# ZHENGXi-git/TC-VIML

Hardware: NVIDIA B200
Metric: linearized_factors_per_s (higher is better)
Workload: dtype f64

## Files before the change

tc-viml_b200/csrc/assemble2.cuh:

```cuda
#pragma once

namespace stream {

constexpr int PMAX = 12;
constexpr int FMAXP = 4096;
constexpr int PT = 64;
constexpr int PT_MAX = 512;
constexpr int TASK_T = 180;
constexpr int TASK_F = 24;
constexpr int LTASK = 32;
constexpr int AW = 4;
constexpr int LACC_W = 14;
constexpr int STAGE_D = 1024;
constexpr int LACC_D = TASK_F * LACC_W;
constexpr int WORK_D = STAGE_D + LACC_D + 192;

struct PlanPtrs {
  int4* hdr;
  int4* tasks;
  uint32_t* slots;
  uint32_t* finfo;
  uint32_t* lslots;
  int* any_irregular;
};

__host__ __device__ inline int task_base(int a0_rel, int w, int F) { return a0_rel / 64 + w * (F / TASK_F + PMAX + 4); }

__device__ __forceinline__ int warp_incl_scan(int v, int lane) {
#pragma unroll
  for (int d = 1; d < 32; d <<= 1) {
    const int t = __shfl_up_sync(0xffffffffu, v, d);
    if (lane >= d) v += t;
  }
  return v;
}

__global__ void __launch_bounds__(PT_MAX) plan_kernel(LinearizeArgs A, PlanPtrs PL) {
  extern __shared__ __align__(16) unsigned char plan_raw[];
  __shared__ int gcount[PMAX + 2], grun[PMAX + 2], lcount[PMAX + 1], lrun[PMAX + 1];
  __shared__ int s_bad, s_big, s_ntasks, s_nlslots;
  const int tid = threadIdx.x, lane = tid & 31, warp = tid >> 5, w = blockIdx.x;
  const int P = A.P, F = A.F, NTH = (int)blockDim.x;
  uint32_t* fmask = reinterpret_cast<uint32_t*>(plan_raw);
  uint32_t* fanchor = fmask + F;
  uint32_t* cexcl = fanchor + F;
  uint16_t* ford = reinterpret_cast<uint16_t*>(cexcl + F + 1);
  uint16_t* fid = ford + ((F + 1) & ~1);
  const int a0 = A.pf_window_offset[w], nf = A.pf_window_offset[w + 1] - a0;
  const int b0 = A.NL > 0 ? A.lf_window_offset[w] : 0, nl = A.NL > 0 ? A.lf_window_offset[w + 1] - b0 : 0;
  const int a0r = a0 - (int)A.pf_begin, b0r = b0 - (int)A.lf_begin;
  for (int f = tid; f < F; f += NTH) fmask[f] = 0u, fanchor[f] = 0xffu;
  for (int e = tid; e < F * P; e += NTH) fid[e] = 0xffff;
  if (tid < PMAX + 2) gcount[tid] = 0;
  if (tid < PMAX + 1) lcount[tid] = 0;
  if (tid == 0) s_bad = s_big = (nf > 65534 || nl > 65534 || nf < 0 || nl < 0) ? 1 : 0, s_ntasks = 0, s_nlslots = 0;
  __syncthreads();
  const int nfs = s_big ? 0 : nf;
  for (int k = tid; k < nfs; k += NTH) {
    const uint32_t ix = A.pf_idx[a0 + k];
    const int i = ix & 0xff, j = (ix >> 8) & 0xff, l = ix >> 16;
    if (i >= P || j >= P || l >= F || i == j) {
      s_bad = 1;
      continue;
    }
    const uint32_t old = atomicOr(&fmask[l], 1u << j);
    const uint32_t an = atomicCAS(&fanchor[l], 0xffu, (uint32_t)i);
    if (((old >> j) & 1u) || (an != 0xffu && an != (uint32_t)i)) s_bad = 1;
    fid[l * P + j] = (uint16_t)k;
  }
  __syncthreads();
  if (s_bad) {
    if (tid == 0) {
      PL.hdr[w] = make_int4(0, 0, 1, 0);
      atomicOr(PL.any_irregular, 1);
    }
    return;
  }
  uint32_t* lsl = PL.lslots + 2 * (size_t)b0r;
  if (warp == 0) {
    for (int f0 = 0; f0 < F; f0 += 32) {
      const int f = f0 + lane;
      const int key = f < F ? (fanchor[f] == 0xffu ? P : (int)fanchor[f]) : 64 + lane;
      const unsigned m = __match_any_sync(0xffffffffu, key);
      if (f < F && (m & ((1u << lane) - 1u)) == 0u) gcount[key] += __popc(m);
      __syncwarp();
    }
    {
      const int c = lane <= P ? gcount[lane] : 0;
      const int inc = warp_incl_scan(c, lane);
      if (lane <= P) grun[lane] = inc - c;
    }
    __syncwarp();
    for (int f0 = 0; f0 < F; f0 += 32) {
      const int f = f0 + lane;
      const int key = f < F ? (fanchor[f] == 0xffu ? P : (int)fanchor[f]) : 64 + lane;
      const unsigned m = __match_any_sync(0xffffffffu, key);
      const int rank = __popc(m & ((1u << lane) - 1u));
      if (f < F) ford[grun[key] + rank] = (uint16_t)f;
      __syncwarp();
      if (f < F && rank == 0) grun[key] += __popc(m);
      __syncwarp();
    }
    int carry = 0;
    for (int p0 = 0; p0 < F; p0 += 32) {
      const int p = p0 + lane;
      const int c = p < F ? __popc(fmask[ford[p]]) : 0;
      const int inc = warp_incl_scan(c, lane);
      if (p < F) cexcl[p] = (uint32_t)(carry + inc - c);
      carry += __shfl_sync(0xffffffffu, inc, 31);
    }
    if (lane == 0) cexcl[F] = (uint32_t)carry;
    __syncwarp();
    const int tb = task_base(a0r, w, F);
    int pos = 0, t = 0;
    bool at_group_start = true;
    while (pos < F) {
      const int p = pos + lane;
      const int c = p < F ? (int)(cexcl[p + 1] - cexcl[p]) : 0x10000;
      const int inc = warp_incl_scan(c, lane);
      const unsigned okm = __ballot_sync(0xffffffffu, inc <= TASK_T && p < F && lane < TASK_F);
      int n = okm == 0xffffffffu ? 32 : __ffs(~okm) - 1;
      n = max(n, 1);
      n = min(n, F - pos);
      const int an = p < F ? (fanchor[ford[p]] == 0xffu ? P : (int)fanchor[ford[p]]) : -1;
      const unsigned same = __ballot_sync(0xffffffffu, an == __shfl_sync(0xffffffffu, an, 0));
      const int na = same == 0xffffffffu ? 33 : __ffs(~same) - 1;
      int excl = 0;
      if (na <= n) {
        n = na;
        excl = at_group_start ? 1 : 0;
        at_group_start = true;
      } else {
        at_group_start = false;
      }
      if (lane == 0) PL.tasks[tb + t] = make_int4(2 * (int)cexcl[pos], 0, pos, n | (excl << 16));
      pos += n, ++t;
    }
    if (lane == 0) s_ntasks = t;
  } else if (warp == 1 && nl > 0) {
    bool bad = false;
    for (int k0 = 0; k0 < nl; k0 += 32) {
      const int k = k0 + lane;
      int key = k < nl ? A.lf_frame[b0 + k] : 64 + lane;
      if (k < nl && (key < 0 || key >= P)) bad = true, key = 96 + lane;
      const unsigned m = __match_any_sync(0xffffffffu, key);
      if (k < nl && key < P && (m & ((1u << lane) - 1u)) == 0u) lcount[key] += __popc(m);
      __syncwarp();
    }
    if (__any_sync(0xffffffffu, bad)) {
      if (lane == 0) s_bad = 1;
    } else {
      const int c = lane < P ? ((lcount[lane] + 1) & ~1) : 0;
      const int inc = warp_incl_scan(c, lane);
      if (lane < P) {
        lrun[lane] = inc - c;
        if (lcount[lane] & 1) lsl[inc - 1] = 0xffffu | ((uint32_t)lane << 16);
      }
      if (lane == 31) s_nlslots = inc;
      __syncwarp();
      for (int k0 = 0; k0 < nl; k0 += 32) {
        const int k = k0 + lane;
        const int key = k < nl ? A.lf_frame[b0 + k] : 64 + lane;
        const unsigned m = __match_any_sync(0xffffffffu, key);
        const int rank = __popc(m & ((1u << lane) - 1u));
        if (k < nl) lsl[lrun[key] + rank] = (uint32_t)k | ((uint32_t)key << 16);
        __syncwarp();
        if (k < nl && rank == 0) lrun[key] += __popc(m);
        __syncwarp();
      }
    }
  }
  __syncthreads();
  if (s_bad) {
    if (tid == 0) {
      PL.hdr[w] = make_int4(0, 0, 1, 0);
      atomicOr(PL.any_irregular, 1);
    }
    return;
  }
  const int tb = task_base(a0r, w, F), nt = s_ntasks;
  uint32_t* sl_w = PL.slots + 2 * (size_t)a0r;
  for (int t = warp; t < nt; t += NTH / 32) {
    int4 tk = PL.tasks[tb + t];
    const int p = tk.z + lane;
    const bool on = lane < (tk.w & 0xffff);
    const int l = on ? ford[p] : 0;
    const uint32_t m = on ? fmask[l] : 0u;
    const int an = (on && m) ? (int)fanchor[l] : 0xff;
    if (on) PL.finfo[(size_t)w * F + p] = (uint32_t)l | (m << 16) | ((uint32_t)(an & 15) << 28);
    uint32_t* sl = sl_w + tk.x;
    int off = 0;
    const unsigned lt = (1u << lane) - 1u;
    unsigned im = __reduce_or_sync(0xffffffffu, an < P ? 1u << an : 0u);
    while (im) {
      const int i = __ffs(im) - 1;
      im &= im - 1;
      unsigned jm = __reduce_or_sync(0xffffffffu, an == i ? m : 0u);
      while (jm) {
        const int j = __ffs(jm) - 1;
        jm &= jm - 1;
        const bool mine = an == i && ((m >> j) & 1u);
        const unsigned b = __ballot_sync(0xffffffffu, mine);
        const int n = __popc(b);
        const uint32_t key = ((uint32_t)i << 21) | ((uint32_t)j << 25);
        if (mine) sl[off + __popc(b & lt)] = (uint32_t)fid[l * P + j] | ((uint32_t)lane << 16) | key;
        if ((n & 1) && lane == 0) sl[off + n] = 0xffffu | key;
        off += (n + 1) & ~1;
      }
    }
    if (lane == 0) PL.tasks[tb + t].y = off;
  }
  if (tid == 0) PL.hdr[w] = make_int4(nt, s_nlslots, 0, 0);
}

enum Kind { K_LL = 0, K_HH, K_LH, K_LE, K_HE, K_EE, K_BL, K_BH, K_BE, K_NKIND };

struct Tables {
  uint32_t seg[128];
  uint32_t lo[64];
  uint32_t ee[32];
  uint32_t line[32];
};

constexpr uint32_t tab_entry(int R, int C, int kind, int off, bool neg) {
  const int tile = (R < 8 && C < 8) ? 0 : (R < 8 ? 1 : 2);
  return 0x80000000u | (uint32_t)(tile * 64 + (R & 7) * 8 + (C & 7)) | ((uint32_t)kind << 8) | ((uint32_t)off << 12) |
         (neg ? (1u << 18) : 0u);
}

constexpr int col_type(int c) { return c < 3 ? 0 : (c < 6 ? 1 : (c < 9 ? 2 : (c < 15 ? 3 : 4))); }
constexpr int col_sub(int c) { return c < 3 ? c : (c < 6 ? c - 3 : (c < 9 ? c - 6 : (c < 15 ? c - 9 : 0))); }

constexpr Tables make_tables() {
  Tables T{};
  int ns = 0, nlo = 0, nli = 0, nee = 0;
  constexpr int kind_order[K_NKIND] = {K_LL, K_LE, K_BL, K_EE, K_BE, K_HH, K_HE, K_BH, K_LH};
  for (int ko = 0; ko < K_NKIND; ++ko)
    for (int off = 0; off < 36; ++off) {
      const int kind = kind_order[ko];
      const bool vec = kind >= K_BL;
      if (vec && off >= 6) continue;
      const int dr = vec ? off : off / 6, dc = vec ? 0 : off % 6;
      for (int R = 0; R < 16; ++R)
        for (int C = R; C < 16; ++C) {
          const int tr = col_type(R), tc = col_type(C), r = col_sub(R), c = col_sub(C);
          bool hit = false, neg = false;
          if (tr == 0 && tc == 0) {
            if (kind == K_LL || kind == K_HH) hit = dr == r && dc == c;
            if (kind == K_LH) hit = dr == r && dc == c, neg = true;
          } else if (tr == 0 && tc == 1) {
            if (kind == K_LL) hit = dr == r && dc == 3 + c;
            if (kind == K_LH) hit = dr == 3 + c && dc == r, neg = true;
          } else if (tr == 0 && tc == 2) {
            if (kind == K_LH) hit = dr == r && dc == 3 + c;
            if (kind == K_HH) hit = dr == r && dc == 3 + c, neg = true;
          } else if (tr == 0 && tc == 3) {
            if (kind == K_LE) hit = dr == r && dc == c;
            if (kind == K_HE) hit = dr == r && dc == c, neg = true;
          } else if (tr == 0 && tc == 4) {
            if (kind == K_BL) hit = dr == r;
            if (kind == K_BH) hit = dr == r, neg = true;
          } else if (tr == 1 && tc == 1) {
            if (kind == K_LL) hit = dr == 3 + r && dc == 3 + c;
          } else if (tr == 1 && tc == 2) {
            if (kind == K_LH) hit = dr == 3 + r && dc == 3 + c;
          } else if (tr == 1 && tc == 3) {
            if (kind == K_LE) hit = dr == 3 + r && dc == c;
          } else if (tr == 1 && tc == 4) {
            if (kind == K_BL) hit = dr == 3 + r;
          } else if (tr == 2 && tc == 2) {
            if (kind == K_HH) hit = dr == 3 + r && dc == 3 + c;
          } else if (tr == 2 && tc == 3) {
            if (kind == K_HE) hit = dr == 3 + r && dc == c;
          } else if (tr == 2 && tc == 4) {
            if (kind == K_BH) hit = dr == 3 + r;
          } else if (tr == 3 && tc == 3) {
            if (kind == K_EE) hit = dr == r && dc == c;
          } else if (tr == 3 && tc == 4) {
            if (kind == K_BE) hit = dr == r;
          }
          if (!hit) continue;
          const bool per_segment = kind == K_HH || kind == K_LH || kind == K_HE || kind == K_BH;
          if (per_segment) {
            T.seg[ns++] = tab_entry(R, C, kind, off, neg);
          } else if (kind == K_EE || kind == K_BE) {
            T.ee[nee++] = tab_entry(R, C, kind, off, neg);
          } else {
            T.lo[nlo++] = tab_entry(R, C, kind, off, neg);
          }
        }
    }
  for (int r = 0; r < 6; ++r)
    for (int c = r; c < 6; ++c) T.line[nli++] = tab_entry(r, c, K_LL, r * 6 + c, false);
  for (int r = 0; r < 6; ++r) T.line[nli++] = tab_entry(r, 6, K_BL, r, false);
  return T;
}
__device__ const Tables g_tables = make_tables();
static_assert(make_tables().seg[95] != 0u && make_tables().seg[96] == 0u, "63 hi-role + 33 (lo, hi) per-segment destinations = three full rounds");
static_assert(make_tables().lo[62] != 0u && make_tables().lo[63] == 0u, "63 per-anchor destinations");
static_assert(make_tables().ee[26] != 0u && make_tables().ee[27] == 0u, "27 extrinsic destinations");
static_assert(make_tables().line[26] != 0u && make_tables().line[27] == 0u, "27 line destinations");


__device__ __forceinline__ void dmma(double& d0, double& d1, double a, double b) {
  asm volatile("mma.sync.aligned.m8n8k4.row.col.f64.f64.f64.f64 {%0,%1}, {%2}, {%3}, {%0,%1};"
               : "+d"(d0), "+d"(d1)
               : "d"(a), "d"(b));
}

__device__ __forceinline__ int blk(int br, int bc, int NB) { return br * NB - (br * (br - 1)) / 2 + (bc - br); }

__device__ __forceinline__ int swz(int f) { return ((f & 1) << 2) ^ ((f >> 1) & 3); }

struct Dest {
  int src;
  int off;
  int kind;
  unsigned sign;
};
__device__ __forceinline__ Dest decode(uint32_t e) {
  Dest d;
  d.src = (e >> 31) ? (int)(e & 0xff) : -1;
  d.off = (e >> 12) & 63;
  d.kind = (e >> 8) & 15;
  d.sign = ((e >> 18) & 1u) << 31;
  return d;
}
template <int ROUNDS>
__device__ __forceinline__ void scatter(const double* __restrict__ patch, const Dest* tab, double* __restrict__ Hc,
                                        int mybase, bool store_lh = false) {
  double v[ROUNDS];
  double* dst[ROUNDS];
#pragma unroll
  for (int r = 0; r < ROUNDS; ++r) {
    const int base = __shfl_sync(0xffffffffu, mybase, tab[r].kind);
    dst[r] = Hc + base + tab[r].off;
    const double x = patch[tab[r].src >= 0 ? tab[r].src : 0];
    v[r] = __hiloint2double(__double2hiint(x) ^ (int)tab[r].sign, __double2loint(x));
  }
#pragma unroll
  for (int r = 0; r < ROUNDS; ++r) {
    if (tab[r].src >= 0) {
      if (store_lh && tab[r].kind == K_LH) *dst[r] = v[r];
      else atomicAdd(dst[r], v[r]);
    }
  }
}

__device__ __forceinline__ int kind_base(int rs, int cs, bool isb, int lo, int hi, int NB, int boff) {
  const int e = NB - 1;
  const int x = rs == 0 ? lo : (rs == 1 ? hi : e), y = cs == 0 ? lo : (cs == 1 ? hi : e);
  return isb ? boff + 6 * x : blk(x, y, NB) * 36;
}

__device__ __forceinline__ void put_patch(double* __restrict__ patch, int lane, const double (&G)[6]) {
  double2* p2 = reinterpret_cast<double2*>(patch);
  const int o = (lane >> 2) * 4 + (lane & 3);
  p2[o] = make_double2(G[0], G[1]);
  p2[32 + o] = make_double2(G[2], G[3]);
  p2[64 + o] = make_double2(G[4], G[5]);
}

template <bool MODE_A>
__global__ void __maxnreg__(168) assemble_kernel(LinearizeArgs A, PlanPtrs PL, int use_tma) {
  extern __shared__ __align__(16) unsigned char asm_raw[];
  __shared__ int s_next;
// ... 418 lines not shown
```

tc-viml_b200/csrc/linearize_kernels.cu:

```cuda
#include <cstdlib>
#include <vector>

#include "common.cuh"

namespace {

__device__ __forceinline__ void quat_to_rot(double w, double x, double y, double z, double* R) {
  const double tx = 2.0 * x, ty = 2.0 * y, tz = 2.0 * z;
  const double twx = tx * w, twy = ty * w, twz = tz * w;
  const double txx = tx * x, txy = ty * x, txz = tz * x;
  const double tyy = ty * y, tyz = tz * y, tzz = tz * z;
  R[0] = 1.0 - (tyy + tzz);
  R[1] = txy - twz;
  R[2] = txz + twy;
  R[3] = txy + twz;
  R[4] = 1.0 - (txx + tzz);
  R[5] = tyz - twx;
  R[6] = txz - twy;
  R[7] = tyz + twx;
  R[8] = 1.0 - (txx + tyy);
}

__device__ __forceinline__ void mul_AtBt(const double* A, const double* B, double* C) {
#pragma unroll
// ... 303 lines not shown
    for (int c = 0; c < 6; ++c) {
      const double v = X[0][r] * Y[0][c] + X[1][r] * Y[1][c];
      atomicAdd(H + (size_t)(r0 + r) * D + c0 + c, v);
      if (!diag) atomicAdd(H + (size_t)(c0 + c) * D + r0 + r, v);
    }
}

__device__ __forceinline__ void point_atomics(const LinearizeArgs& A, int w, int i, int j, int f, const PointJac& J, bool live,
                                              bool warp_window) {
  const int D = A.D;
  double* H = A.out.H_pp + (size_t)w * D * D;
  double* bp = A.out.b_p + (size_t)w * D;
  const int oi = 6 * i, oj = 6 * j, oe = 6 * A.P;
  if (warp_window) {
    double v[27];
    int n = 0;
#pragma unroll
    for (int r = 0; r < 6; ++r)
#pragma unroll
      for (int c = r; c < 6; ++c) v[n++] = live ? J.c[0][r] * J.c[0][c] + J.c[1][r] * J.c[1][c] : 0.0;
#pragma unroll
    for (int r = 0; r < 6; ++r) v[21 + r] = live ? J.c[0][r] * J.r[0] + J.c[1][r] * J.r[1] : 0.0;
#pragma unroll
    for (int e = 0; e < 27; ++e)
#pragma unroll
      for (int d = 16; d > 0; d >>= 1) v[e] += __shfl_xor_sync(0xffffffffu, v[e], d);
    if ((threadIdx.x & 31) == 0) {
      n = 0;
#pragma unroll
      for (int r = 0; r < 6; ++r)
#pragma unroll
        for (int c = r; c < 6; ++c) {
          atomicAdd(H + (size_t)(oe + r) * D + oe + c, v[n]);
          if (c != r) atomicAdd(H + (size_t)(oe + c) * D + oe + r, v[n]);
          ++n;
        }
#pragma unroll
      for (int r = 0; r < 6; ++r) atomicAdd(bp + oe + r, v[21 + r]);
    }
  }
  if (!live) return;
  double* Hl = A.out.H_lp + ((size_t)w * A.F + f) * D;
  atomic_block(H, D, oi, oi, J.a, J.a, true);
  atomic_block(H, D, oi, oj, J.a, J.b, false);
  atomic_block(H, D, oi, oe, J.a, J.c, false);
  atomic_block(H, D, oj, oj, J.b, J.b, true);
  atomic_block(H, D, oj, oe, J.b, J.c, false);
  if (!warp_window) atomic_block(H, D, oe, oe, J.c, J.c, true);
#pragma unroll
  for (int r = 0; r < 6; ++r) {
    atomicAdd(bp + oi + r, J.a[0][r] * J.r[0] + J.a[1][r] * J.r[1]);
    atomicAdd(bp + oj + r, J.b[0][r] * J.r[0] + J.b[1][r] * J.r[1]);
    if (!warp_window) atomicAdd(bp + oe + r, J.c[0][r] * J.r[0] + J.c[1][r] * J.r[1]);
    atomicAdd(Hl + oi + r, J.a[0][r] * J.d[0] + J.a[1][r] * J.d[1]);
    atomicAdd(Hl + oj + r, J.b[0][r] * J.d[0] + J.b[1][r] * J.d[1]);
    atomicAdd(Hl + oe + r, J.c[0][r] * J.d[0] + J.c[1][r] * J.d[1]);
  }
  atomicAdd(A.out.H_ll + (size_t)w * A.F + f, J.d[0] * J.d[0] + J.d[1] * J.d[1]);
  atomicAdd(A.out.b_l + (size_t)w * A.F + f, J.d[0] * J.r[0] + J.d[1] * J.r[1]);
}

__device__ __forceinline__ void line_atomics(const LinearizeArgs& A, int w, int frame, const LineJac& J) {
  const int D = A.D;
  double* H = A.out.H_pp + (size_t)w * D * D;
  double* bp = A.out.b_p + (size_t)w * D;
  const int of = 6 * frame;
  atomic_block(H, D, of, of, J.a, J.a, true);
#pragma unroll
  for (int r = 0; r < 6; ++r) atomicAdd(bp + of + r, J.a[0][r] * J.r[0] + J.a[1][r] * J.r[1]);
}

template <bool MODE_A, bool MODE_B>
#ifndef VIML_POINTS_MINB
#define VIML_POINTS_MINB 4
#endif
__global__ void __launch_bounds__(128, MODE_B ? 2 : VIML_POINTS_MINB) points_kernel(LinearizeArgs A) {
  __shared__ double2 stage[MODE_A ? 4 * 7 * 32 : 1];
  const int64_t k_raw = A.pf_begin + blockIdx.x * (int64_t)blockDim.x + threadIdx.x;
  const int64_t k_end = A.pf_begin + A.NP;
  const int lane = threadIdx.x & 31;
  const int64_t k_warp = k_raw - lane;
  if (k_warp >= k_end) return;
  const int nvalid = (int)min((int64_t)32, k_end - k_warp);
  const int64_t k = min(k_raw, k_end - 1);
  const bool live = k_raw < k_end;
  const int w = find_window_warp(A.pf_window_offset, A.W, k, k_warp);
  const uint32_t pk = A.pf_idx[k];
  const int i = pk & 0xff, j = (pk >> 8) & 0xff, f = pk >> 16;
  const double4 ob = reinterpret_cast<const double4*>(A.pf_obs)[k];
  const double piz = A.pf_pts_i_z ? A.pf_pts_i_z[k] : 1.0;
  const double lam = A.inv_depth[(size_t)w * A.F + f];
  const double* cw = A.cache + (size_t)w * (A.P * kPoseCache + kExCache);
  PointJac J;
  eval_point(A, cw, i, j, lam, ob.x, ob.y, piz, ob.z, ob.w, J);
  if (MODE_A) {
    double2* st = stage + (threadIdx.x >> 5) * 7 * 32;
    if (live && A.out.pf_residual) reinterpret_cast<double2*>(A.out.pf_residual)[k] = make_double2(J.r[0], J.r[1]);
    if (A.out.pf_jac_pose_i) store_jac7_coalesced(st, A.out.pf_jac_pose_i + 14 * k_warp, J.a, lane, nvalid);
    if (A.out.pf_jac_pose_j) store_jac7_coalesced(st, A.out.pf_jac_pose_j + 14 * k_warp, J.b, lane, nvalid);
    if (A.out.pf_jac_ex) store_jac7_coalesced(st, A.out.pf_jac_ex + 14 * k_warp, J.c, lane, nvalid);
    if (live && A.out.pf_jac_feat) reinterpret_cast<double2*>(A.out.pf_jac_feat)[k] = make_double2(J.d[0], J.d[1]);
  }
  if (MODE_B) {
    const bool warp_window = __all_sync(0xffffffffu, w == __shfl_sync(0xffffffffu, w, 0));
    point_atomics(A, w, i, j, f, J, live, warp_window);
  }
}

template <bool MODE_A, bool MODE_B>
__global__ void __launch_bounds__(128) lines_kernel(LinearizeArgs A) {
  __shared__ double2 stage[MODE_A ? 4 * 7 * 32 : 1];
  const int64_t k_raw = A.lf_begin + blockIdx.x * (int64_t)blockDim.x + threadIdx.x;
  const int64_t k_end = A.lf_begin + A.NL;
  const int lane = threadIdx.x & 31;
  const int64_t k_warp = k_raw - lane;
  if (k_warp >= k_end) return;
  const int nvalid = (int)min((int64_t)32, k_end - k_warp);
  const int64_t k = min(k_raw, k_end - 1);
  const bool live = k_raw < k_end;
  const int w = find_window_warp(A.lf_window_offset, A.W, k, k_warp);
  const int frame = A.lf_frame[k];
  double g9[9];
#pragma unroll
  for (int c = 0; c < 9; ++c) g9[c] = A.lf_geom[(size_t)c * A.NL_stride + k];
  const double* cw = A.cache + (size_t)w * (A.P * kPoseCache + kExCache);
  LineJac J;
  eval_line(A, cw, frame, g9, J);
  if (MODE_A) {
    if (live && A.out.lf_residual) reinterpret_cast<double2*>(A.out.lf_residual)[k] = make_double2(J.r[0], J.r[1]);
    if (A.out.lf_jac_pose)
      store_jac7_coalesced(stage + (threadIdx.x >> 5) * 7 * 32, A.out.lf_jac_pose + 14 * k_warp, J.a, lane, nvalid);
  }
  if (MODE_B && live) line_atomics(A, w, frame, J);
}

__global__ void __launch_bounds__(256) pack_upper_kernel(int D, const double* __restrict__ S, double* __restrict__ Sp) {
  const double* __restrict__ s = S + (size_t)blockIdx.x * D * D;
  double* __restrict__ o = Sp + (size_t)blockIdx.x * ((size_t)D * (D + 1) / 2);
  for (int e = blockIdx.y * blockDim.x + threadIdx.x; e < D * D; e += gridDim.y * blockDim.x) {
    const int r = e / D, c = e - r * D;
    if (c >= r) o[(size_t)r * D - ((size_t)r * (r - 1)) / 2 + c - r] = s[e];
  }
}

#include "assemble2.cuh"
#include "gn_kernels.cuh"

}

int viml_launch_linearize(viml_ctx* ctx, const LinearizeArgs& a) {
  cudaStream_t st = ctx->stream;
  const bool modeA = (a.flags & VIML_OUT_RESIDUAL_JACOBIAN) != 0;
  const bool modeB = (a.flags & (VIML_OUT_HB | VIML_OUT_SCHUR)) != 0;
  const size_t plan_smem = (size_t)a.F * 8 + ((size_t)a.F + 1) * 4 + (((size_t)a.F + 1) & ~(size_t)1) * 2 + (size_t)a.F * a.P * 2 + 16;
  const bool fast = modeB && a.P <= stream::PMAX && a.F <= stream::FMAXP && plan_smem <= 200 * 1024 && !ctx->force_generic;
  stream::PlanPtrs PL{};
  if (fast) {
    const size_t n_tasks = (size_t)a.NP / 64 + (size_t)a.W * (a.F / stream::TASK_F + stream::PMAX + 4) + 2;
    auto pad = [](size_t b) { return DeviceArena::padded(b); };
    VIML_TRY_CUDA(ctx, ctx->scratch3.reserve(pad((size_t)a.W * 16) + pad(n_tasks * 16) + pad((size_t)a.NP * 8 + 8) +
                                             pad((size_t)a.W * a.F * 4 + 4) + pad((size_t)a.NL * 8 + 8) + pad(4)));
    PL.hdr = ctx->scratch3.take<int4>((size_t)a.W);
    PL.tasks = ctx->scratch3.take<int4>(n_tasks);
    PL.slots = ctx->scratch3.take<uint32_t>((size_t)a.NP * 2 + 2);
    PL.finfo = ctx->scratch3.take<uint32_t>((size_t)a.W * a.F + 1);
    PL.lslots = ctx->scratch3.take<uint32_t>((size_t)a.NL * 2 + 2);
    PL.any_irregular = ctx->scratch3.take<int>(1);
    VIML_TRY_CUDA(ctx, cudaEventRecord(ctx->ev_fork, st));
    VIML_TRY_CUDA(ctx, cudaStreamWaitEvent(ctx->aux_stream, ctx->ev_fork, 0));
    VIML_TRY_CUDA(ctx, cudaMemsetAsync(PL.any_irregular, 0, 4, ctx->aux_stream));
    VIML_TRY_CUDA(ctx, cudaFuncSetAttribute(stream::plan_kernel, cudaFuncAttributeMaxDynamicSharedMemorySize, (int)plan_smem));
    {
      LaunchScope ls(ctx, K_PLAN, ctx->aux_stream);
      stream::plan_kernel<<<a.W, a.F > 512 ? stream::PT_MAX : stream::PT, plan_smem, ctx->aux_stream>>>(a, PL);
    }
    VIML_TRY_CUDA(ctx, cudaEventRecord(ctx->ev_join, ctx->aux_stream));
  }
  {
    const int64_t total = (int64_t)a.W * (a.P + 1);
    LaunchScope ls(ctx, K_PREP);
    prep_windows_kernel<<<(unsigned)((total + 127) / 128), 128, 0, st>>>(a);
  }
  if (fast) {
    VIML_TRY_CUDA(ctx, cudaStreamWaitEvent(st, ctx->ev_join, 0));
    const int NB = a.P + 1, nblk = NB * (NB + 1) / 2;
    const size_t smem = ((size_t)((nblk * 36 + a.D + 1) & ~1) + (size_t)a.P * kPoseCache + kExCache + (size_t)stream::AW * stream::WORK_D) * 8;
    const int use_tma = ((((uintptr_t)a.out.H_pp) | ((uintptr_t)a.out.b_p)) & 15) == 0 ? 1 : 0;
    VIML_TRY_CUDA(ctx, cudaFuncSetAttribute(stream::assemble_kernel<true>, cudaFuncAttributeMaxDynamicSharedMemorySize, (int)smem));
    VIML_TRY_CUDA(ctx, cudaFuncSetAttribute(stream::assemble_kernel<false>, cudaFuncAttributeMaxDynamicSharedMemorySize, (int)smem));
    {
      LaunchScope ls(ctx, K_ASSEMBLE);
      if (modeA) stream::assemble_kernel<true><<<a.W, stream::AW * 32, smem, st>>>(a, PL, use_tma);
      else stream::assemble_kernel<false><<<a.W, stream::AW * 32, smem, st>>>(a, PL, use_tma);
    }
    {
      const int grid = a.W < 4 * ctx->sm_count ? a.W : 4 * ctx->sm_count;
      LaunchScope ls(ctx, K_IRREGULAR);
      if (modeA) stream::irregular_kernel<true><<<grid, 128, 0, st>>>(a, PL);
      else stream::irregular_kernel<false><<<grid, 128, 0, st>>>(a, PL);
    }
  } else {
    if (modeB) {
      const size_t W = a.W, D = a.D, F = a.F;
      VIML_TRY_CUDA(ctx, cudaMemsetAsync(a.out.H_pp, 0, W * D * D * sizeof(double), st));
      VIML_TRY_CUDA(ctx, cudaMemsetAsync(a.out.H_lp, 0, W * F * D * sizeof(double), st));
      VIML_TRY_CUDA(ctx, cudaMemsetAsync(a.out.H_ll, 0, W * F * sizeof(double), st));
      VIML_TRY_CUDA(ctx, cudaMemsetAsync(a.out.b_p, 0, W * D * sizeof(double), st));
      VIML_TRY_CUDA(ctx, cudaMemsetAsync(a.out.b_l, 0, W * F * sizeof(double), st));
    }
    if (a.NP > 0) {
      const unsigned grid = (unsigned)((a.NP + 127) / 128);
      LaunchScope ls(ctx, K_POINTS);
      if (modeA && modeB) points_kernel<true, true><<<grid, 128, 0, st>>>(a);
      else if (modeA) points_kernel<true, false><<<grid, 128, 0, st>>>(a);
      else if (modeB) points_kernel<false, true><<<grid, 128, 0, st>>>(a);
    }
    if (a.NL > 0) {
      const unsigned grid = (unsigned)((a.NL + 127) / 128);
      LaunchScope ls(ctx, K_LINES);
      if (modeA && modeB) lines_kernel<true, true><<<grid, 128, 0, st>>>(a);
      else if (modeA) lines_kernel<true, false><<<grid, 128, 0, st>>>(a);
      else if (modeB) lines_kernel<false, true><<<grid, 128, 0, st>>>(a);
    }
  }
  if (a.flags & VIML_OUT_SCHUR) {
    const double eps = 1e-8;
    double* S = a.out.S;
    if (a.flags & VIML_S_PACKED) {
      VIML_TRY_CUDA(ctx, ctx->s_full.reserve(DeviceArena::padded((size_t)a.W * a.D * a.D * 8)));
      S = ctx->s_full.take<double>((size_t)a.W * a.D * a.D);
    }
    viml_launch_schur(ctx, a.W, a.F, a.D, a.out.H_pp, a.out.H_lp, a.out.H_ll, a.out.b_p, a.out.b_l, S, a.out.g, eps);
    if (a.flags & VIML_S_PACKED) {
      LaunchScope ls(ctx, K_SCHUR);
      const unsigned slices = (unsigned)std::min<int64_t>(((int64_t)a.D * a.D + 256 * 32 - 1) / (256 * 32), 1024);
      pack_upper_kernel<<<dim3((unsigned)a.W, slices), 256, 0, st>>>(a.D, S, a.out.S);
    }
  }
  VIML_TRY_CUDA(ctx, cudaGetLastError());
  return VIML_OK;
}

int viml_launch_expand_obs(viml_ctx* ctx, const LinearizeArgs& a, const void* feat_obs, const void* pf_obs_j, bool f32) {
  if (a.NP == 0) return VIML_OK;
  LaunchScope ls(ctx, K_PREP);
  if (f32) expand_obs_kernel<float2><<<a.W, 128, 0, ctx->stream>>>(a, (const float2*)feat_obs, (const float2*)pf_obs_j);
  else expand_obs_kernel<double2><<<a.W, 128, 0, ctx->stream>>>(a, (const double2*)feat_obs, (const double2*)pf_obs_j);
  VIML_TRY_CUDA(ctx, cudaGetLastError());
  return VIML_OK;
}

int viml_launch_expand_lines(viml_ctx* ctx, const LinearizeArgs& a, const int32_t* lf_map_index, const float* lf_seg2d) {
  if (a.NL == 0) return VIML_OK;
  if (!ctx->map_set || ctx->n_map <= 0) {
    ctx->err = "line factors given by map index need a map (viml_set_map)";
    return VIML_ERR_NOMAP;
  }
  MapFrame mf;
  for (int k = 0; k < 9; ++k) mf.R[k] = ctx->cfg.Rbw[k];
  for (int k = 0; k < 3; ++k) mf.T[k] = ctx->cfg.Tbw[k];
  LaunchScope ls(ctx, K_PREP);
  expand_lines_kernel<<<(unsigned)((a.NL + 127) / 128), 128, 0, ctx->stream>>>(a, ctx->d_map, ctx->n_map, mf, lf_map_index,
                                                                             reinterpret_cast<const float4*>(lf_seg2d));
  VIML_TRY_CUDA(ctx, cudaGetLastError());
  return VIML_OK;
}

int viml_launch_prep(viml_ctx* ctx, const LinearizeArgs& a) {
  const int64_t total = (int64_t)a.W * (a.P + 1);
  LaunchScope ls(ctx, K_PREP);
  prep_windows_kernel<<<(unsigned)((total + 127) / 128), 128, 0, ctx->stream>>>(a);
  VIML_TRY_CUDA(ctx, cudaGetLastError());
  return VIML_OK;
}

int viml_launch_reduced(viml_ctx* ctx, int W, int D, const DenseArgs& dn, const double* S, const double* g, double* Sx, double* gx) {
  LaunchScope ls(ctx, K_GN);
  const int smem = gn::kReducedStage * (int)sizeof(double);
  VIML_TRY_CUDA(ctx, cudaFuncSetAttribute(gn::reduced_kernel, cudaFuncAttributeMaxDynamicSharedMemorySize, smem));
  gn::reduced_kernel<<<W, 256, smem, ctx->stream>>>(D, dn, S, g, Sx, gx);
  VIML_TRY_CUDA(ctx, cudaGetLastError());
  return VIML_OK;
}

int viml_launch_gn_solve(viml_ctx* ctx, int W, int Dx, double lambda, const double* Sx, const double* gx, double* dx, int32_t* solved,
                         double* cost) {
  const int NB = (Dx + 7) / 8;
  const size_t smem_t = ((size_t)NB * (NB + 1) / 2 * 64 + (size_t)NB * 8) * sizeof(double);
  LaunchScope ls(ctx, K_GN);
  if (smem_t <= 220 * 1024 && Dx <= 256 - 8 && !getenv("VIML_GN_UNBLOCKED")) {
    VIML_TRY_CUDA(ctx, cudaFuncSetAttribute(gn::solve_tiled_kernel<false>, cudaFuncAttributeMaxDynamicSharedMemorySize, (int)smem_t));
    gn::solve_tiled_kernel<false><<<W, 256, smem_t, ctx->stream>>>(Dx, lambda, Sx, gx, dx, solved, cost, 0, DenseArgs{}, nullptr, nullptr);
    VIML_TRY_CUDA(ctx, cudaGetLastError());
    return VIML_OK;
  }
  const size_t smem = ((size_t)Dx * (Dx + 1) / 2 + Dx) * sizeof(double);
  VIML_TRY_CUDA(ctx, cudaFuncSetAttribute(gn::solve_kernel, cudaFuncAttributeMaxDynamicSharedMemorySize, (int)smem));
  gn::solve_kernel<<<W, 256, smem, ctx->stream>>>(Dx, lambda, Sx, gx, dx, solved, cost);
  VIML_TRY_CUDA(ctx, cudaGetLastError());
  return VIML_OK;
}

int viml_launch_gn_reduced_solve(viml_ctx* ctx, int W, int D, const DenseArgs& dn, const double* S, const double* g, double lambda,
                                 double* dx, int32_t* solved, double* cost) {
  const int Dx = D + dn.X, NB = (Dx + 7) / 8;
  const size_t smem = ((size_t)NB * (NB + 1) / 2 * 64 + 3 * (size_t)NB * 8 + gn::kFusedStage) * sizeof(double);
  if (smem > 224 * 1024 || Dx > 256 - 8 || getenv("VIML_GN_UNBLOCKED") || getenv("VIML_GN_UNFUSED")) return VIML_ERR_UNSUPPORTED;
  LaunchScope ls(ctx, K_GN);
  VIML_TRY_CUDA(ctx, cudaFuncSetAttribute(gn::solve_tiled_kernel<true>, cudaFuncAttributeMaxDynamicSharedMemorySize, (int)smem));
  gn::solve_tiled_kernel<true><<<W, 256, smem, ctx->stream>>>(Dx, lambda, nullptr, nullptr, dx, solved, cost, D, dn, S, g);
  VIML_TRY_CUDA(ctx, cudaGetLastError());
  return VIML_OK;
}

int viml_launch_gn_update(viml_ctx* ctx, const LinearizeArgs& a, int X, const double* extra_in, const double* dx, const int32_t* solved,
                          double* o_poses, double* o_ex, double* o_dep, double* o_extra) {
  LaunchScope ls(ctx, K_GN);
  gn::update_kernel<<<a.W, 128, 0, ctx->stream>>>(a, X, extra_in, dx, solved, o_poses, o_ex, o_dep, o_extra);
  VIML_TRY_CUDA(ctx, cudaGetLastError());
  return VIML_OK;
}

int viml_launch_cost(viml_ctx* ctx, const LinearizeArgs& a, const DenseArgs& dn, const double* dx, int slot, double* cost) {
  LaunchScope ls(ctx, K_GN);
  gn::cost_kernel<<<a.W, 128, 0, ctx->stream>>>(a, dn, dx, slot, cost);
  VIML_TRY_CUDA(ctx, cudaGetLastError());
  return VIML_OK;
// ... 2 lines not shown
```

Measured before the change: 5.495 billion.

## Restructure plan kernel to parallelize grouping, ordering and task building across warps

New measurement: 5.610 billion (median of 6 runs). 2.1% higher.

```diff
diff --git a/profiles/plan_time.py b/profiles/plan_time.py
--- /dev/null
+++ b/profiles/plan_time.py
@@ -0,0 +1,76 @@
+import argparse
+import json
+import os
+import subprocess
+import sys
+
+ROOT = os.path.dirname(os.path.dirname(os.path.abspath(__file__)))
+sys.path.insert(0, ROOT)
+import numpy as np
+import torch
+
+import __graft_entry__ as ge
+from bench import tile_batch
+
+KERNELS = ("plan_windows", "prep_windows", "assemble_hb", "assemble_irregular")
+
+
+def card():
+    q = subprocess.run(["nvidia-smi", "--query-gpu=name,power.limit,clocks.max.sm", "--format=csv,noheader"],
+                       capture_output=True, text=True)
+    return q.stdout.strip().splitlines()[0] if q.returncode == 0 and q.stdout.strip() else "unknown"
+
+
+def time_step(pkg, ctx, batch, steps, warm=5):
+    abi = pkg._abi
+    stream = torch.cuda.ExternalStream(ctx.stream())
+    d_in = {k: ctx.to_device(v) for k, v in batch.arrays().items() if v is not None}
+    shapes = batch.out_shapes()
+    d_out = {k: ctx.device_alloc(int(np.prod(shapes[k])) * 8) for k in ("H_pp", "H_lp", "H_ll", "b_p", "b_l")}
+    s_in, s_out = batch.struct(d_in), abi.out_struct(d_out)
+    flags = abi.OUT_HB | abi.LOSS_CAUCHY | abi.PTRS_DEVICE
+
+    def call():
+        ctx.linearize_raw(s_in, s_out, flags)
+    for _ in range(warm):
+        call()
+    ctx.sync()
+    e0, e1 = torch.cuda.Event(enable_timing=True), torch.cuda.Event(enable_timing=True)
+    ctx.profile_begin()
+    e0.record(stream)
+    for _ in range(steps):
+        call()
+    e1.record(stream)
+    prof = ctx.profile_end()
+    e1.synchronize()
+    for p in list(d_in.values()) + list(d_out.values()):
+        ctx.device_free(p)
+    r = {"step_ms": e0.elapsed_time(e1) / steps}
+    r.update({k: prof[k][0] / steps for k in KERNELS if k in prof})
+    return r
+
+
+def main():
+    ap = argparse.ArgumentParser()
+    ap.add_argument("--steps", type=int, default=50)
+    ap.add_argument("--json")
+    args = ap.parse_args()
+    pkg = ge.load_package()
+    synth = pkg.synth
+    cfg = synth.euroc_config()
+    res = {"card": card(), "library": pkg.LIB_PATH, "steps": args.steps, "unit": "ms per call", "shapes": {}}
+    with pkg.Context(cfg, device=0) as ctx:
+        b4096, _ = synth.with_line_map(synth.make_windows(4096, seed=0x5EED + 2, f32_obs=True), cfg)
+        res["shapes"]["cfg2_1024"] = time_step(pkg, ctx, b4096.slice_windows(0, 1024), args.steps)
+        res["shapes"]["cfg2_4096"] = time_step(pkg, ctx, b4096, args.steps)
+        res["shapes"]["cfg2_65536"] = time_step(pkg, ctx, tile_batch(pkg._abi, b4096, 16), max(5, args.steps // 10))
+        b4 = tile_batch(pkg._abi, synth.make_windows(256, seed=0x5EED + 4, P=11, F=2000, all_start_zero=True, lines_per_frame=0), 16)
+        res["shapes"]["cfg4_4096"] = time_step(pkg, ctx, b4, max(5, args.steps // 5))
+    print(json.dumps(res, indent=1))
+    if args.json:
+        with open(args.json, "w") as f:
+            json.dump(res, f, indent=1)
+
+
+if __name__ == "__main__":
+    main()
diff --git a/tc-viml_b200/csrc/assemble2.cuh b/tc-viml_b200/csrc/assemble2.cuh
--- a/tc-viml_b200/csrc/assemble2.cuh
+++ b/tc-viml_b200/csrc/assemble2.cuh
@@ -1,217 +1,15 @@
 #pragma once
 
+#include "plan.cuh"
+
 namespace stream {
 
-constexpr int PMAX = 12;
-constexpr int FMAXP = 4096;
-constexpr int PT = 64;
-constexpr int PT_MAX = 512;
-constexpr int TASK_T = 180;
-constexpr int TASK_F = 24;
 constexpr int LTASK = 32;
 constexpr int AW = 4;
 constexpr int LACC_W = 14;
 constexpr int STAGE_D = 1024;
 constexpr int LACC_D = TASK_F * LACC_W;
 constexpr int WORK_D = STAGE_D + LACC_D + 192;
-
-struct PlanPtrs {
-  int4* hdr;
-  int4* tasks;
-  uint32_t* slots;
-  uint32_t* finfo;
-  uint32_t* lslots;
-  int* any_irregular;
-};
-
-__host__ __device__ inline int task_base(int a0_rel, int w, int F) { return a0_rel / 64 + w * (F / TASK_F + PMAX + 4); }
-
-__device__ __forceinline__ int warp_incl_scan(int v, int lane) {
-#pragma unroll
-  for (int d = 1; d < 32; d <<= 1) {
-    const int t = __shfl_up_sync(0xffffffffu, v, d);
-    if (lane >= d) v += t;
-  }
-  return v;
-}
-
-__global__ void __launch_bounds__(PT_MAX) plan_kernel(LinearizeArgs A, PlanPtrs PL) {
-  extern __shared__ __align__(16) unsigned char plan_raw[];
-  __shared__ int gcount[PMAX + 2], grun[PMAX + 2], lcount[PMAX + 1], lrun[PMAX + 1];
-  __shared__ int s_bad, s_big, s_ntasks, s_nlslots;
-  const int tid = threadIdx.x, lane = tid & 31, warp = tid >> 5, w = blockIdx.x;
-  const int P = A.P, F = A.F, NTH = (int)blockDim.x;
-  uint32_t* fmask = reinterpret_cast<uint32_t*>(plan_raw);
-  uint32_t* fanchor = fmask + F;
-  uint32_t* cexcl = fanchor + F;
-  uint16_t* ford = reinterpret_cast<uint16_t*>(cexcl + F + 1);
-  uint16_t* fid = ford + ((F + 1) & ~1);
-  const int a0 = A.pf_window_offset[w], nf = A.pf_window_offset[w + 1] - a0;
-  const int b0 = A.NL > 0 ? A.lf_window_offset[w] : 0, nl = A.NL > 0 ? A.lf_window_offset[w + 1] - b0 : 0;
-  const int a0r = a0 - (int)A.pf_begin, b0r = b0 - (int)A.lf_begin;
-  for (int f = tid; f < F; f += NTH) fmask[f] = 0u, fanchor[f] = 0xffu;
-  for (int e = tid; e < F * P; e += NTH) fid[e] = 0xffff;
-  if (tid < PMAX + 2) gcount[tid] = 0;
-  if (tid < PMAX + 1) lcount[tid] = 0;
-  if (tid == 0) s_bad = s_big = (nf > 65534 || nl > 65534 || nf < 0 || nl < 0) ? 1 : 0, s_ntasks = 0, s_nlslots = 0;
-  __syncthreads();
-  const int nfs = s_big ? 0 : nf;
-  for (int k = tid; k < nfs; k += NTH) {
-    const uint32_t ix = A.pf_idx[a0 + k];
-    const int i = ix & 0xff, j = (ix >> 8) & 0xff, l = ix >> 16;
-    if (i >= P || j >= P || l >= F || i == j) {
-      s_bad = 1;
-      continue;
-    }
-    const uint32_t old = atomicOr(&fmask[l], 1u << j);
-    const uint32_t an = atomicCAS(&fanchor[l], 0xffu, (uint32_t)i);
-    if (((old >> j) & 1u) || (an != 0xffu && an != (uint32_t)i)) s_bad = 1;
-    fid[l * P + j] = (uint16_t)k;
-  }
-  __syncthreads();
-  if (s_bad) {
-    if (tid == 0) {
-      PL.hdr[w] = make_int4(0, 0, 1, 0);
-      atomicOr(PL.any_irregular, 1);
-    }
-    return;
-  }
-  uint32_t* lsl = PL.lslots + 2 * (size_t)b0r;
-  if (warp == 0) {
-    for (int f0 = 0; f0 < F; f0 += 32) {
-      const int f = f0 + lane;
-      const int key = f < F ? (fanchor[f] == 0xffu ? P : (int)fanchor[f]) : 64 + lane;
-      const unsigned m = __match_any_sync(0xffffffffu, key);
-      if (f < F && (m & ((1u << lane) - 1u)) == 0u) gcount[key] += __popc(m);
-      __syncwarp();
-    }
-    {
-      const int c = lane <= P ? gcount[lane] : 0;
-      const int inc = warp_incl_scan(c, lane);
-      if (lane <= P) grun[lane] = inc - c;
-    }
-    __syncwarp();
-    for (int f0 = 0; f0 < F; f0 += 32) {
-      const int f = f0 + lane;
-      const int key = f < F ? (fanchor[f] == 0xffu ? P : (int)fanchor[f]) : 64 + lane;
-      const unsigned m = __match_any_sync(0xffffffffu, key);
-      const int rank = __popc(m & ((1u << lane) - 1u));
-      if (f < F) ford[grun[key] + rank] = (uint16_t)f;
-      __syncwarp();
-      if (f < F && rank == 0) grun[key] += __popc(m);
-      __syncwarp();
-    }
-    int carry = 0;
-    for (int p0 = 0; p0 < F; p0 += 32) {
-      const int p = p0 + lane;
-      const int c = p < F ? __popc(fmask[ford[p]]) : 0;
-      const int inc = warp_incl_scan(c, lane);
-      if (p < F) cexcl[p] = (uint32_t)(carry + inc - c);
-      carry += __shfl_sync(0xffffffffu, inc, 31);
-    }
-    if (lane == 0) cexcl[F] = (uint32_t)carry;
-    __syncwarp();
-    const int tb = task_base(a0r, w, F);
-    int pos = 0, t = 0;
-    bool at_group_start = true;
-    while (pos < F) {
-      const int p = pos + lane;
-      const int c = p < F ? (int)(cexcl[p + 1] - cexcl[p]) : 0x10000;
-      const int inc = warp_incl_scan(c, lane);
-      const unsigned okm = __ballot_sync(0xffffffffu, inc <= TASK_T && p < F && lane < TASK_F);
-      int n = okm == 0xffffffffu ? 32 : __ffs(~okm) - 1;
-      n = max(n, 1);
-      n = min(n, F - pos);
-      const int an = p < F ? (fanchor[ford[p]] == 0xffu ? P : (int)fanchor[ford[p]]) : -1;
-      const unsigned same = __ballot_sync(0xffffffffu, an == __shfl_sync(0xffffffffu, an, 0));
-      const int na = same == 0xffffffffu ? 33 : __ffs(~same) - 1;
-      int excl = 0;
-      if (na <= n) {
-        n = na;
-        excl = at_group_start ? 1 : 0;
-        at_group_start = true;
-      } else {
-        at_group_start = false;
-      }
-      if (lane == 0) PL.tasks[tb + t] = make_int4(2 * (int)cexcl[pos], 0, pos, n | (excl << 16));
-      pos += n, ++t;
-    }
-    if (lane == 0) s_ntasks = t;
-  } else if (warp == 1 && nl > 0) {
-    bool bad = false;
-    for (int k0 = 0; k0 < nl; k0 += 32) {
-      const int k = k0 + lane;
-      int key = k < nl ? A.lf_frame[b0 + k] : 64 + lane;
-      if (k < nl && (key < 0 || key >= P)) bad = true, key = 96 + lane;
-      const unsigned m = __match_any_sync(0xffffffffu, key);
-      if (k < nl && key < P && (m & ((1u << lane) - 1u)) == 0u) lcount[key] += __popc(m);
-      __syncwarp();
-    }
-    if (__any_sync(0xffffffffu, bad)) {
-      if (lane == 0) s_bad = 1;
-    } else {
-      const int c = lane < P ? ((lcount[lane] + 1) & ~1) : 0;
-      const int inc = warp_incl_scan(c, lane);
-      if (lane < P) {
-        lrun[lane] = inc - c;
-        if (lcount[lane] & 1) lsl[inc - 1] = 0xffffu | ((uint32_t)lane << 16);
-      }
-      if (lane == 31) s_nlslots = inc;
-      __syncwarp();
-      for (int k0 = 0; k0 < nl; k0 += 32) {
-        const int k = k0 + lane;
-        const int key = k < nl ? A.lf_frame[b0 + k] : 64 + lane;
-        const unsigned m = __match_any_sync(0xffffffffu, key);
-        const int rank = __popc(m & ((1u << lane) - 1u));
-        if (k < nl) lsl[lrun[key] + rank] = (uint32_t)k | ((uint32_t)key << 16);
-        __syncwarp();
-        if (k < nl && rank == 0) lrun[key] += __popc(m);
-        __syncwarp();
-      }
-    }
-  }
-  __syncthreads();
-  if (s_bad) {
-    if (tid == 0) {
-      PL.hdr[w] = make_int4(0, 0, 1, 0);
-      atomicOr(PL.any_irregular, 1);
-    }
-    return;
-  }
-  const int tb = task_base(a0r, w, F), nt = s_ntasks;
-  uint32_t* sl_w = PL.slots + 2 * (size_t)a0r;
-  for (int t = warp; t < nt; t += NTH / 32) {
-    int4 tk = PL.tasks[tb + t];
-    const int p = tk.z + lane;
-    const bool on = lane < (tk.w & 0xffff);
-    const int l = on ? ford[p] : 0;
-    const uint32_t m = on ? fmask[l] : 0u;
-    const int an = (on && m) ? (int)fanchor[l] : 0xff;
-    if (on) PL.finfo[(size_t)w * F + p] = (uint32_t)l | (m << 16) | ((uint32_t)(an & 15) << 28);
-    uint32_t* sl = sl_w + tk.x;
-    int off = 0;
-    const unsigned lt = (1u << lane) - 1u;
-    unsigned im = __reduce_or_sync(0xffffffffu, an < P ? 1u << an : 0u);
-    while (im) {
-      const int i = __ffs(im) - 1;
-      im &= im - 1;
-      unsigned jm = __reduce_or_sync(0xffffffffu, an == i ? m : 0u);
-      while (jm) {
-        const int j = __ffs(jm) - 1;
-        jm &= jm - 1;
-        const bool mine = an == i && ((m >> j) & 1u);
-        const unsigned b = __ballot_sync(0xffffffffu, mine);
-        const int n = __popc(b);
-        const uint32_t key = ((uint32_t)i << 21) | ((uint32_t)j << 25);
-        if (mine) sl[off + __popc(b & lt)] = (uint32_t)fid[l * P + j] | ((uint32_t)lane << 16) | key;
-        if ((n & 1) && lane == 0) sl[off + n] = 0xffffu | key;
-        off += (n + 1) & ~1;
-      }
-    }
-    if (lane == 0) PL.tasks[tb + t].y = off;
-  }
-  if (tid == 0) PL.hdr[w] = make_int4(nt, s_nlslots, 0, 0);
-}
 
 enum Kind { K_LL = 0, K_HH, K_LH, K_LE, K_HE, K_EE, K_BL, K_BH, K_BE, K_NKIND };
 
diff --git a/tc-viml_b200/csrc/linearize_kernels.cu b/tc-viml_b200/csrc/linearize_kernels.cu
--- a/tc-viml_b200/csrc/linearize_kernels.cu
+++ b/tc-viml_b200/csrc/linearize_kernels.cu
@@ -479,7 +479,7 @@
   cudaStream_t st = ctx->stream;
   const bool modeA = (a.flags & VIML_OUT_RESIDUAL_JACOBIAN) != 0;
   const bool modeB = (a.flags & (VIML_OUT_HB | VIML_OUT_SCHUR)) != 0;
-  const size_t plan_smem = (size_t)a.F * 8 + ((size_t)a.F + 1) * 4 + (((size_t)a.F + 1) & ~(size_t)1) * 2 + (size_t)a.F * a.P * 2 + 16;
+  const size_t plan_smem = stream::plan_smem_bytes(a.P, a.F);
   const bool fast = modeB && a.P <= stream::PMAX && a.F <= stream::FMAXP && plan_smem <= 200 * 1024 && !ctx->force_generic;
   stream::PlanPtrs PL{};
   if (fast) {
@@ -496,10 +496,9 @@
     VIML_TRY_CUDA(ctx, cudaEventRecord(ctx->ev_fork, st));
     VIML_TRY_CUDA(ctx, cudaStreamWaitEvent(ctx->aux_stream, ctx->ev_fork, 0));
     VIML_TRY_CUDA(ctx, cudaMemsetAsync(PL.any_irregular, 0, 4, ctx->aux_stream));
-    VIML_TRY_CUDA(ctx, cudaFuncSetAttribute(stream::plan_kernel, cudaFuncAttributeMaxDynamicSharedMemorySize, (int)plan_smem));
     {
       LaunchScope ls(ctx, K_PLAN, ctx->aux_stream);
-      stream::plan_kernel<<<a.W, a.F > 512 ? stream::PT_MAX : stream::PT, plan_smem, ctx->aux_stream>>>(a, PL);
+      VIML_TRY_CUDA(ctx, stream::launch_plan(a, PL, ctx->aux_stream));
     }
     VIML_TRY_CUDA(ctx, cudaEventRecord(ctx->ev_join, ctx->aux_stream));
   }
diff --git a/tc-viml_b200/csrc/plan.cuh b/tc-viml_b200/csrc/plan.cuh
--- /dev/null
+++ b/tc-viml_b200/csrc/plan.cuh
@@ -0,0 +1,254 @@
+#pragma once
+
+namespace stream {
+
+constexpr int PMAX = 12;
+constexpr int FMAXP = 4096;
+constexpr int PT = 64;
+constexpr int PT_MAX = 512;
+constexpr int PU = 12;
+constexpr int LU = 4;
+constexpr int TASK_T = 180;
+constexpr int TASK_F = 24;
+
+struct PlanPtrs {
+  int4* hdr;
+  int4* tasks;
+  uint32_t* slots;
+  uint32_t* finfo;
+  uint32_t* lslots;
+  int* any_irregular;
+};
+
+__host__ __device__ inline int task_base(int a0_rel, int w, int F) { return a0_rel / 64 + w * (F / TASK_F + PMAX + 4); }
+
+__device__ __forceinline__ int warp_incl_scan(int v, int lane) {
+#pragma unroll
+  for (int d = 1; d < 32; d <<= 1) {
+    const int t = __shfl_up_sync(0xffffffffu, v, d);
+    if (lane >= d) v += t;
+  }
+  return v;
+}
+
+__host__ __device__ inline size_t plan_smem_bytes(int P, int F) {
+  const size_t NC = ((size_t)F + 31) / 32;
+  return ((size_t)3 * F + 1 + (size_t)(P + 1) * NC) * 4 + (((size_t)F + 1) & ~(size_t)1) * 2 + (size_t)F * P * 2;
+}
+
+template <int NTH>
+__global__ void __launch_bounds__(NTH, 2048 / NTH) plan_kernel(LinearizeArgs A, PlanPtrs PL) {
+  constexpr int NW = NTH / 32;
+  constexpr unsigned full = 0xffffffffu;
+  extern __shared__ __align__(16) unsigned char plan_raw[];
+  __shared__ int kbase[PMAX + 2];
+  __shared__ int ntk[PMAX + 1];
+  __shared__ int wsum[NW];
+  __shared__ int lcount[PMAX], lrun[PMAX];
+  __shared__ int s_bad, s_nlslots;
+  const int tid = threadIdx.x, lane = tid & 31, warp = tid >> 5, w = blockIdx.x;
+  const unsigned lt = (1u << lane) - 1u;
+  const int P = A.P, F = A.F, NC = (F + 31) >> 5;
+  uint32_t* fword = reinterpret_cast<uint32_t*>(plan_raw);
+  uint32_t* cex = fword + F;
+  uint32_t* tlist = cex + F + 1;
+  uint32_t* ccnt = tlist + F;
+  uint16_t* ford = reinterpret_cast<uint16_t*>(ccnt + (P + 1) * NC);
+  uint16_t* fid = ford + ((F + 1) & ~1);
+
+  const int a0 = A.pf_window_offset[w], nf = A.pf_window_offset[w + 1] - a0;
+  const int b0 = A.NL > 0 ? A.lf_window_offset[w] : 0, nl = A.NL > 0 ? A.lf_window_offset[w + 1] - b0 : 0;
+  const int a0r = a0 - (int)A.pf_begin, b0r = b0 - (int)A.lf_begin;
+  const bool big = nf > 65534 || nl > 65534 || nf < 0 || nl < 0;
+  const int nfs = big ? 0 : nf, nls = big ? 0 : nl;
+  const int lwarp = nls > 0 ? NW - 1 : NW;
+  uint32_t ix[PU];
+#pragma unroll
+  for (int u = 0; u < PU; ++u) ix[u] = tid + u * NTH < nfs ? A.pf_idx[a0 + tid + u * NTH] : 0u;
+  int lfr[LU];
+#pragma unroll
+  for (int u = 0; u < LU; ++u) lfr[u] = warp == lwarp && u * 32 + lane < nls ? A.lf_frame[b0 + u * 32 + lane] : 0;
+  for (int f = tid; f < F; f += NTH) fword[f] = 0u;
+  for (int e = tid; e < (P + 1) * NC; e += NTH) ccnt[e] = 0u;
+  if (tid < PMAX) lcount[tid] = 0;
+  if (tid == 0) s_bad = big ? 1 : 0, s_nlslots = 0;
+  __syncthreads();
+
+  for (int k0 = 0;;) {
+#pragma unroll
+    for (int u = 0; u < PU; ++u) {
+      const int k = k0 + tid + u * NTH;
+      if (k < nfs) {
+        const int i = ix[u] & 0xff, j = (ix[u] >> 8) & 0xff, l = ix[u] >> 16;
+        if (i >= P || j >= P || l >= F || i == j) {
+          s_bad = 1;
+        } else {
+          const uint32_t old = atomicOr(&fword[l], (1u << j) | (1u << (16 + i)));
+          if ((old >> j) & 1u) s_bad = 1;
+          fid[l * P + j] = (uint16_t)k;
+        }
+      }
+    }
+    k0 += PU * NTH;
+    if (k0 >= nfs) break;
+#pragma unroll
+    for (int u = 0; u < PU; ++u) ix[u] = k0 + tid + u * NTH < nfs ? A.pf_idx[a0 + k0 + tid + u * NTH] : 0u;
+  }
+  __syncthreads();
+
+  if (warp < lwarp) {
+    for (int c = warp; c < NC; c += lwarp) {
+      const int f = c * 32 + lane;
+      const uint32_t am = f < F ? fword[f] >> 16 : 0u;
+      if (__popc(am) > 1) s_bad = 1;
+      const int key = f < F ? (am ? __ffs(am) - 1 : P) : 64 + lane;
+      const unsigned m = __match_any_sync(full, key);
+      if (f < F && (m & lt) == 0u) ccnt[key * NC + c] = __popc(m);
+    }
+  } else if (warp == lwarp) {
+    bool bad = false;
+    auto count = [&](int k, int fr) {
+      int key = k < nls ? fr : 64 + lane;
+      if (k < nls && (key < 0 || key >= P)) bad = true, key = 96 + lane;
+      const unsigned m = __match_any_sync(full, key);
+      if (k < nls && key < P && (m & lt) == 0u) lcount[key] += __popc(m);
+      __syncwarp();
+    };
+#pragma unroll
+    for (int u = 0; u < LU; ++u)
+      if (u * 32 < nls) count(u * 32 + lane, lfr[u]);
+    for (int k0 = LU * 32; k0 < nls; k0 += 32) count(k0 + lane, k0 + lane < nls ? A.lf_frame[b0 + k0 + lane] : 0);
+    if (__any_sync(full, bad)) {
+      if (lane == 0) s_bad = 1;
+    } else {
+      const int c = lane < P ? ((lcount[lane] + 1) & ~1) : 0;
+      const int inc = warp_incl_scan(c, lane);
+      if (lane < P) lrun[lane] = inc - c;
+      if (lane == 31) s_nlslots = inc;
+    }
+  }
+  __syncthreads();
+  if (s_bad) {
+    if (tid == 0) {
+      PL.hdr[w] = make_int4(0, 0, 1, 0);
+      atomicOr(PL.any_irregular, 1);
+    }
+    return;
+  }
+
+  if (warp == 0) {
+    int run = 0;
+    if (lane <= P)
+      for (int c = 0; c < NC; ++c) {
+        const int v = (int)ccnt[lane * NC + c];
+        ccnt[lane * NC + c] = (uint32_t)run;
+        run += v;
+      }
+    const int inc = warp_incl_scan(lane <= P ? run : 0, lane);
+    if (lane <= P) kbase[lane] = inc - run;
+    if (lane == P) kbase[P + 1] = inc;
+  } else if (warp == lwarp) {
+    uint32_t* lsl = PL.lslots + 2 * (size_t)b0r;
+    if (lane < P && (lcount[lane] & 1)) lsl[lrun[lane] + lcount[lane]] = 0xffffu | ((uint32_t)lane << 16);
+    __syncwarp();
+    auto place = [&](int k, int fr) {
+      const int key = k < nls ? fr : 64 + lane;
+      const unsigned m = __match_any_sync(full, key);
+      const int rank = __popc(m & lt);
+      if (k < nls) lsl[lrun[key] + rank] = (uint32_t)k | ((uint32_t)key << 16);
+      __syncwarp();
+      if (k < nls && rank == 0) lrun[key] += __popc(m);
+      __syncwarp();
+    };
+#pragma unroll
+    for (int u = 0; u < LU; ++u)
+      if (u * 32 < nls) place(u * 32 + lane, lfr[u]);
+    for (int k0 = LU * 32; k0 < nls; k0 += 32) place(k0 + lane, k0 + lane < nls ? A.lf_frame[b0 + k0 + lane] : 0);
+  }
+  __syncthreads();
+
+  for (int c = warp; c < NC; c += NW) {
+    const int f = c * 32 + lane;
+    const uint32_t am = f < F ? fword[f] >> 16 : 0u;
+    const int key = f < F ? (am ? __ffs(am) - 1 : P) : 64 + lane;
+    const unsigned m = __match_any_sync(full, key);
+    if (f < F) ford[kbase[key] + (int)ccnt[key * NC + c] + __popc(m & lt)] = (uint16_t)f;
+  }
+  __syncthreads();
+
+  {
+    const int R = (F + NTH - 1) / NTH, p0 = min(F, tid * R), p1 = min(F, p0 + R);
+    int s = 0;
+    for (int p = p0; p < p1; ++p) s += __popc(fword[ford[p]] & 0xfffu);
+    const int inc = warp_incl_scan(s, lane);
+    if (lane == 31) wsum[warp] = inc;
+    __syncthreads();
+    int run = inc - s;
+    for (int q = 0; q < warp; ++q) run += wsum[q];
+    for (int p = p0; p < p1; ++p) {
+      cex[p] = (uint32_t)run;
+      run += __popc(fword[ford[p]] & 0xfffu);
+    }
+    if (tid == NTH - 1) cex[F] = (uint32_t)run;
+  }
+  __syncthreads();
+
+  for (int g = warp; g <= P; g += NW) {
+    const int gs = kbase[g], ge = kbase[g + 1];
+    int pos = gs, t = 0;
+    while (pos < ge) {
+      const int p = pos + lane;
+      const bool ok = lane < TASK_F && p < ge && (int)(cex[p + 1] - cex[pos]) <= TASK_T;
+      const int n = max(1, __popc(__ballot_sync(full, ok)));
+      if (lane == 0) tlist[gs + t] = (uint32_t)pos | ((uint32_t)n << 16) | ((pos == gs && pos + n == ge) ? 1u << 24 : 0u);
+      pos += n, ++t;
+    }
+    if (lane == 0) ntk[g] = t;
+  }
+  __syncthreads();
+
+  const int v = lane <= P ? ntk[lane] : 0;
+  const int tinc = warp_incl_scan(v, lane);
+  const int nt = __shfl_sync(full, tinc, P);
+  if (tid == 0) PL.hdr[w] = make_int4(nt, s_nlslots, 0, 0);
+  const int tb = task_base(a0r, w, F);
+  uint32_t* sl_w = PL.slots + 2 * (size_t)a0r;
+  for (int t = warp; t < nt; t += NW) {
+    const int g = __popc(__ballot_sync(full, lane <= P && tinc <= t));
+    const int tg = __shfl_sync(full, tinc - v, g);
+    const uint32_t e = tlist[kbase[g] + t - tg];
+    const int pos = e & 0xffff, n = (e >> 16) & 0xff;
+    const bool on = lane < n;
+    const int l = on ? ford[pos + lane] : 0;
+    const uint32_t m = on ? fword[l] & 0xfffu : 0u;
+    if (on) PL.finfo[(size_t)w * F + pos + lane] = (uint32_t)l | (m << 16) | ((uint32_t)(m ? g : 15) << 28);
+    const int x = 2 * (int)cex[pos];
+    uint32_t* sl = sl_w + x;
+    int off = 0;
+    unsigned jm = __reduce_or_sync(full, m);
+    while (jm) {
+      const int j = __ffs(jm) - 1;
+      jm &= jm - 1;
+      const bool mine = (m >> j) & 1u;
+      const unsigned b = __ballot_sync(full, mine);
+      const int nn = __popc(b);
+      const uint32_t key = ((uint32_t)g << 21) | ((uint32_t)j << 25);
+      if (mine) sl[off + __popc(b & lt)] = (uint32_t)fid[l * P + j] | ((uint32_t)lane << 16) | key;
+      if ((nn & 1) && lane == 0) sl[off + nn] = 0xffffu | key;
+      off += (nn + 1) & ~1;
+    }
+    if (lane == 0) PL.tasks[tb + t] = make_int4(x, off, pos, n | (int)((e >> 24) << 16));
+  }
+}
+
+inline cudaError_t launch_plan(const LinearizeArgs& a, const PlanPtrs& PL, cudaStream_t st) {
+  const size_t smem = plan_smem_bytes(a.P, a.F);
+  const bool many = a.F > 512;
+  auto k = many ? plan_kernel<PT_MAX> : plan_kernel<PT>;
+  cudaError_t e = cudaFuncSetAttribute(k, cudaFuncAttributeMaxDynamicSharedMemorySize, (int)smem);
+  if (e != cudaSuccess) return e;
+  k<<<a.W, many ? PT_MAX : PT, smem, st>>>(a, PL);
+  return cudaGetLastError();
+}
+
+}
```
